# feiyeha/EGM-Unet

Measured on AMD Instinct MI355X. Metric: train images/sec at 3x512x512 bs=8/GPU, higher is better.
Workload: dtype bf16; 1 GPU; EGM-UNet GRFBUNet(3,2,base_c=32) fwd+5-term-loss+bwd+SGD, 8x3x512x512 per GPU (BASELINE.json configs[1]); global_batch=8, parallelism=dp1, launch=hipGraph replay, world_size=1

## Files before the change

### egm_unet_amd/csrc/conv3x3_wreg.hip

```cpp
#include "common.h"
#include "group.h"
#include "bn_elem.h"
#include <stdlib.h>

typedef __attribute__((ext_vector_type(8))) __bf16 bf16x8_t;
typedef __attribute__((ext_vector_type(16))) float f32x16_t;
typedef __attribute__((ext_vector_type(2))) float f32x2_t;
typedef __attribute__((ext_vector_type(2))) __bf16 bf16x2_t;

__device__ uint4 egm_dump_wreg[64];
__device__ uint4 egm_zero_page_wreg[4];

namespace {

constexpr int TW = 32, PW = TW + 2, R = 2, TROWS = 16, PH = TROWS + 2, NBUF = 3;
constexpr int PSLOTS = PH * PW * 4;
constexpr int NPI = (PSLOTS + 63) / 64;
constexpr int KT = (NPI + 7) / 8;
constexpr int STAGE = KT * 8 * 1024;
constexpr int OROW = 64 + 16;
constexpr int SMEM = NBUF * STAGE + 8 * R * 32 * OROW;
static_assert(SMEM <= 160 * 1024, "LDS budget");
static_assert(KT <= 6, "DMA slots of a stage");

struct WregParams {
    const bf16_t* x; const bf16_t* w; const float* bias; bf16_t* y; float* stats;
    int ldx, ldy, N, H, W, Cin, Cout, bias_n;
    int tiles_y, tiles_x, npt, G;
};

__device__ __forceinline__ uint32_t pack2(float lo, float hi) {
    f32x2_t v; v.x = lo; v.y = hi;
    const bf16x2_t b = __builtin_convertvector(v, bf16x2_t);
    return *reinterpret_cast<const uint32_t*>(&b);
}
__device__ __forceinline__ void glds16(const void* gsrc, unsigned lds_byte_addr) {
    unsigned keep;
    asm volatile("s_mov_b32 %0, m0\n\ts_mov_b32 m0, %2\n\ts_nop 0\n\tglobal_load_lds_dwordx4 %1, off\n\ts_mov_b32 m0, %0"
                 : "=&s"(keep) : "v"(gsrc), "s"(lds_byte_addr));
}

template <int CH>
__global__ __launch_bounds__(512, 2) void conv3x3_wreg_kernel(WregParams p) {
    constexpr int ACT = EGM_ACT_NONE;
#include "conv3x3_wreg_body.h"
}
template <int CH, int ACT>
__global__ __launch_bounds__(512, 2) void conv3x3_wreg_act_kernel(WregParams p) {
#include "conv3x3_wreg_body.h"
}

template <int CH, int ACT = EGM_ACT_NONE>
int launch_wreg(const WregParams& p, hipStream_t st) {
    constexpr auto kern = [] { if constexpr (ACT == EGM_ACT_NONE) return &conv3x3_wreg_kernel<CH>; else return &conv3x3_wreg_act_kernel<CH, ACT>; }();
    static bool attr_done = false;
    if (!attr_done) {
        hipError_t e = hipFuncSetAttribute(reinterpret_cast<const void*>(kern), hipFuncAttributeMaxDynamicSharedMemorySize, 160 * 1024);
        if (e != hipSuccess) EGM_FAIL(EGM_ERR_LAUNCH, "conv3x3_wreg: hipFuncSetAttribute: %s", hipGetErrorString(e));
        attr_done = true;
    }
    hipLaunchKernelGGL(kern, dim3(p.G), dim3(512), SMEM, st, p);
    EGM_CHECK_LAUNCH("conv3x3_wreg");
    return EGM_OK;
}
}

int egm_conv_tile_mode(int mode);

int egm_conv_wreg_plan(int dtype, int N, int H, int W, int Cin, int Cout, int KH, int KW, int dil, int* G_out) {
    if (dtype != EGM_BF16 || KH != 3 || KW != 3 || dil != 1 || Cout != 32 || Cin != 32) return 0;
    if (egm_group_recording()) return 0;
    if (!(egm_conv_tile_mode(-1) & 4)) return 0;
    const long long npt = (long long)N * egm_cdiv(H, TROWS) * egm_cdiv(W, TW);
    if (npt < 512) return 0;
    *G_out = 256;
    return 1;
}
const char* egm_conv_wreg_name(int Cin) { (void)Cin; return "conv3x3_wreg_kernel<1>"; }

int egm_conv_wreg_launch(const void* x, int ldx, const void* wf, const float* bias, int bias_n, void* y, int ldy, float* stats, int N, int H,
                         int W, int Cin, int Cout, int G, egm_stream_t s, int act) {
    WregParams p;
    p.x = (const bf16_t*)x; p.w = (const bf16_t*)wf; p.bias = bias; p.y = (bf16_t*)y; p.stats = stats;
    p.ldx = ldx; p.ldy = ldy; p.N = N; p.H = H; p.W = W; p.Cin = Cin; p.Cout = Cout; p.bias_n = bias ? bias_n : 0;
    p.tiles_y = egm_cdiv(H, TROWS); p.tiles_x = egm_cdiv(W, TW); p.npt = N * p.tiles_y * p.tiles_x; p.G = G;
    EGM_REQUIRE((long long)(PH + 1) * W * ldx < (1LL << 31), "conv3x3_wreg: halo window offsets exceed 32 bits");
    switch (act) {
        case EGM_ACT_RELU: return launch_wreg<1, EGM_ACT_RELU>(p, (hipStream_t)s);
        case EGM_ACT_SIGMOID: return launch_wreg<1, EGM_ACT_SIGMOID>(p, (hipStream_t)s);
        case EGM_ACT_SILU: return launch_wreg<1, EGM_ACT_SILU>(p, (hipStream_t)s);
        default: return launch_wreg<1>(p, (hipStream_t)s);
    }
}
```

### egm_unet_amd/csrc/conv_igemm.hip

```cpp
#include "common.h"
#include "group.h"
#include "bn_elem.h"
#include <string.h>
#include <stdio.h>

typedef __attribute__((ext_vector_type(8))) __bf16 bf16x8_t;
typedef __attribute__((ext_vector_type(16))) float f32x16_t;
typedef __attribute__((ext_vector_type(2))) unsigned short u16x2_t;

int egm_conv_direct_plan(int dtype, int N, int H, int W, int Cin, int Cout, int KH, int KW, int dil, int* NT_out, int* nct_out, int* G_out,
                         size_t* smem_out);
int egm_conv_direct_launch(const void* x, int ldx, const void* wf, const float* bias, int bias_n, void* y, int ldy,
                           float* stats, int N, int H, int W, int Cin, int Cout, int KH, int KW, int dil, int NT, int nct, int G, size_t smem,
                           egm_stream_t s, int act = EGM_ACT_NONE);

int egm_conv_tile_plan(int dtype, int N, int H, int W, int Cin, int Cout, int KH, int KW, int dil, int* cfg_out, int* nct_out, int* G_out);
const char* egm_conv_tile_name(int cfg);
int egm_conv_wreg_plan(int dtype, int N, int H, int W, int Cin, int Cout, int KH, int KW, int dil, int* G_out);
const char* egm_conv_wreg_name(int Cin);
int egm_conv_wreg_launch(const void* x, int ldx, const void* wf, const float* bias, int bias_n, void* y, int ldy, float* stats, int N, int H,
                         int W, int Cin, int Cout, int G, egm_stream_t s, int act = EGM_ACT_NONE);
int egm_conv_tile_launch(const void* x, int ldx, const void* wf, const float* bias, int bias_n, void* y, int ldy, float* stats, int N, int H,
                         int W, int Cin, int Cout, int cfg, int nct, int G, egm_stream_t s, void* y2 = nullptr, int ldy2 = 0, int csplit = 0,
                         int act = EGM_ACT_NONE);
int egm_conv_c7_plan(int dtype, int N, int H, int W, int Cin, int Cout, int KH, int KW, int dil);
int egm_conv_c7_launch(const void* x, int ldx, const void* wf, const float* bias, int bias_n, void* y, int ldy, int N, int H, int W,
                       egm_stream_t s, int act = EGM_ACT_NONE);
int egm_conv_c16d_plan(int dtype, int N, int H, int W, int Cin, int Cout, int KH, int KW, int dil);
int egm_conv_c16d_launch(const void* x, int ldx, const void* wf, const float* bias, int bias_n, void* y, int ldy, float* stats, int N, int H,
                         int W, int dil, egm_stream_t s, int act = EGM_ACT_NONE);

namespace {

constexpr int TH = 8, TW = 32, KC = 32;

template <typename T> struct Mma;
template <> struct Mma<bf16_t> {
    static constexpr int kStep = 16;
    static constexpr int kPixStride = KC * 2 + 16;
    using Frag = bf16x8_t;
    static __device__ __forceinline__ Frag load(const unsigned char* row, int ks, int h) {
        return *reinterpret_cast<const Frag*>(row + ks * 32 + h * 16);
    }
    static __device__ __forceinline__ f32x16_t mma(Frag a, Frag b, f32x16_t c) {
        return __builtin_amdgcn_mfma_f32_32x32x16_bf16(a, b, c, 0, 0, 0);
    }
    static __device__ __forceinline__ void stage16(unsigned char* dst, const bf16_t* src, bool ok) {
        uint4 v = make_uint4(0, 0, 0, 0);
        if (ok) v = *reinterpret_cast<const uint4*>(src);
        *reinterpret_cast<uint4*>(dst) = v;
    }
    static __device__ __forceinline__ void stage_val(unsigned char* dst, uint4 v) { *reinterpret_cast<uint4*>(dst) = v; }
};
template <> struct Mma<float> {
// ... 559 lines not shown
    c.R = 2;
    if (c.pipe && KH == 3 && dil == 1 && Cout <= 32) {
        const long long npt4 = (long long)N * egm_cdiv(H, 16) * egm_cdiv(W, TW);
        if (npt4 >= 256) c.R = 4;
    }
    static const int r1_on = getenv("EGM_PIPE_R1") ? atoi(getenv("EGM_PIPE_R1")) : 1;
    if (r1_on && c.pipe && KH == 3 && dil == 1 && c.R == 2 && Cout > 32 && Cin >= 128) {
        const long long wgs2 = (long long)N * egm_cdiv(H, 8) * egm_cdiv(W, TW) * egm_cdiv(Cout, 32);
        if (wgs2 <= 256) c.R = 1;
    }
    c.tiles_y = egm_cdiv(H, 4 * c.R); c.tiles_x = egm_cdiv(W, TW); c.npt = N * c.tiles_y * c.tiles_x;
    c.NT = (c.R == 4) ? (Cout <= 32 ? 1 : 2) : (c.R == 1 ? 1 : conv_nt(c.npt, Cout));
    c.nct = egm_cdiv(Cout, 32 * c.NT);
    if (!c.pipe) { c.G = c.npt; return c; }
    if (c.R == 4) {
        const int per_cu = (c.NT == 2) ? 1 : 2;
        int g = (256 * per_cu / c.nct) / 8 * 8;
        if (g < 8) g = 8;
        if (g > c.npt) g = c.npt;
        c.G = g;
    } else {
        c.G = pipe_groups(c.npt, c.nct);
    }
    return c;
}
}

extern "C" int egm_conv_kernel_name(int dtype, int N, int H, int W, int Cin, int Cout, int KH, int KW, int dil, char* buf, int buflen) {
    if (KH == 1 && KW == 1) dil = 1;
    const ConvPlan c = conv_plan(dtype, N, H, W, Cin, Cout, KH, KW, dil);
    char tmp[96];
    if (c.c16d) snprintf(tmp, sizeof(tmp), "conv3x3d_c16_kernel");
    else if (c.c7) snprintf(tmp, sizeof(tmp), "conv7x7_c16_kernel");
    else if (c.wreg) snprintf(tmp, sizeof(tmp), "%s", egm_conv_wreg_name(Cin));
    else if (c.tile) snprintf(tmp, sizeof(tmp), "%s", egm_conv_tile_name(c.tile_cfg));
    else if (c.direct) snprintf(tmp, sizeof(tmp), "conv_direct_kernel<%d, %s>", c.NT, KH == 1 ? "true" : "false");
    else if (c.pipe) snprintf(tmp, sizeof(tmp), "conv_igemm_pipe_kernel<%d, %d, %d, %d>", c.NT, (KH == 3 && dil == 1) ? 3 : 1,
                              (KH == 3 && dil == 1) ? 3 : (KH == 7 ? 7 : 1), c.R);
    else snprintf(tmp, sizeof(tmp), "conv_igemm_kernel<%s, %d>", dtype == EGM_BF16 ? "bf16_t" : "float", c.NT);
    const int n = (int)strlen(tmp);
    if (buf != nullptr && buflen > 0) { strncpy(buf, tmp, (size_t)buflen - 1); buf[buflen - 1] = 0; }
    return n;
}
extern "C" int egm_conv_stats_tiles(int dtype, int N, int H, int W, int Cin, int Cout, int KH, int KW, int dil) {
    return conv_plan(dtype, N, H, W, Cin, Cout, KH, KW, dil).G;
}

extern "C" int egm_conv_pack(int dtype, const void* w, void* wf, void* wd, int Cout, int Cin, int KH, int KW, int groups,
                             egm_stream_t s) {
    EGM_REQUIRE(w != nullptr && (wf != nullptr || wd != nullptr), "conv_pack: null pointer");
    EGM_REQUIRE(Cout > 0 && Cin > 0 && groups > 0 && Cout % groups == 0 && Cin % groups == 0, "conv_pack: bad channels/groups");
    EGM_REQUIRE(KH > 0 && KW > 0 && (KH & 1) && (KW & 1), "conv_pack: kernel must be odd");
    const int CoutP = (Cout + 7) / 8 * 8, CinP = (Cin + 7) / 8 * 8;
    const long long total = (long long)KH * KW * CoutP * CinP;
    const int grid = (int)((total + 255) / 256 > 4096 ? 4096 : (total + 255) / 256);
    EGM_DISPATCH_DTYPE(dtype, hipLaunchKernelGGL((conv_pack_kernel<T>), dim3(grid), dim3(256), 0, (hipStream_t)s,
                                                 (const float*)w, (T*)wf, (T*)wd, Cout, Cin, CoutP, CinP, KH, KW, groups));
    EGM_CHECK_LAUNCH("conv_pack");
    return EGM_OK;
}

extern "C" int egm_conv_pack_chunk(void) { return kPackChunk; }
extern "C" int egm_conv_pack_multi(int dtype, const void* table_dev, int n, long long total_chunks, egm_stream_t s) {
    EGM_REQUIRE(table_dev && n > 0 && total_chunks > 0 && total_chunks < (1LL << 30), "conv_pack_multi: bad args");
    EGM_DISPATCH_DTYPE(dtype, hipLaunchKernelGGL((conv_pack_multi_kernel<T>), dim3((unsigned)total_chunks), dim3(256), 0, (hipStream_t)s,
                                                 (const PackEntry*)table_dev, n));
    EGM_CHECK_LAUNCH("conv_pack_multi");
    return EGM_OK;
}

extern "C" int egm_conv_split_ok(int dtype, int N, int H, int W, int Cin, int Cout, int KH, int KW, int dil, int csplit) {
    if (csplit <= 0 || csplit >= Cout || csplit % 8 || N <= 0 || H <= 0 || W <= 0 || Cin <= 0 || Cin % 8 || Cout % 8) return 0;
    const ConvPlan c = conv_plan(dtype, N, H, W, Cin, Cout, KH, KW, dil);
    return (!c.c7 && !c.wreg && c.tile) ? 1 : 0;
}
extern "C" int egm_conv_fwd_split(int dtype, const void* x, int ldx, const void* wf, void* y, int ldy, void* y2, int ldy2, int csplit, int N,
                                  int H, int W, int Cin, int Cout, int KH, int KW, int dil, egm_stream_t s) {
    EGM_REQUIRE(x && wf && y && y2 && egm_aligned16(x) && egm_aligned16(wf) && egm_aligned16(y) && egm_aligned16(y2), "conv_fwd_split: bad pointers");
    EGM_REQUIRE(egm_conv_split_ok(dtype, N, H, W, Cin, Cout, KH, KW, dil, csplit), "conv_fwd_split: shape not supported (egm_conv_split_ok)");
    EGM_REQUIRE(ldx >= Cin && ldx % 8 == 0 && ldy >= csplit && ldy % 8 == 0 && ldy2 >= Cout - csplit && ldy2 % 8 == 0, "conv_fwd_split: bad ld");
    const ConvPlan c = conv_plan(dtype, N, H, W, Cin, Cout, KH, KW, dil);
    return egm_conv_tile_launch(x, ldx, wf, nullptr, 0, y, ldy, nullptr, N, H, W, Cin, Cout, c.tile_cfg, c.nct, c.G, s, y2, ldy2, csplit);
}

static int conv_fwd_impl(int dtype, const void* x, int ldx, const void* wf, const void* bias, int bias_n, void* y, int ldy, float* stats,
                         int N, int H, int W, int Cin, int Cout, int KH, int KW, int dil, int act, egm_stream_t s) {
    EGM_REQUIRE(x && wf && y, "conv_fwd: null pointer");
    EGM_REQUIRE(!bias || (bias_n > 0 && bias_n <= Cout), "conv_fwd: bad bias_n %d", bias_n);
    EGM_REQUIRE(N > 0 && H > 0 && W > 0, "conv_fwd: bad shape N=%d H=%d W=%d", N, H, W);
    EGM_REQUIRE(Cin > 0 && Cout > 0 && Cin % 8 == 0 && Cout % 8 == 0, "conv_fwd: Cin=%d/Cout=%d must be multiples of 8", Cin, Cout);
    EGM_REQUIRE(ldx >= Cin && ldy >= Cout && ldx % 8 == 0 && ldy % 8 == 0, "conv_fwd: bad ld (ldx=%d ldy=%d)", ldx, ldy);
    EGM_REQUIRE((KH & 1) && (KW & 1) && KH <= 7 && KW <= 7 && dil >= 1, "conv_fwd: unsupported kernel %dx%d dil %d", KH, KW, dil);
    EGM_REQUIRE(egm_aligned16(x) && egm_aligned16(wf) && egm_aligned16(y), "conv_fwd: pointers must be 16-byte aligned");
    EGM_REQUIRE((long long)N * H * W * (long long)(ldx > ldy ? ldx : ldy) < (1LL << 40), "conv_fwd: tensor too large");
    if (KH == 1 && KW == 1) dil = 1;

    ConvParams p;
    p.x = x; p.w = wf; p.bias = (const float*)bias; p.y = y; p.stats = stats;
    p.ldx = ldx; p.ldy = ldy; p.N = N; p.H = H; p.W = W; p.Cin = Cin; p.Cout = Cout; p.KH = KH; p.KW = KW; p.dil = dil; p.bias_n = bias ? bias_n : 0;
    p.wl = egm_w_layout(dtype, KH, KW, Cin, Cout);
    const ConvPlan c = conv_plan(dtype, N, H, W, Cin, Cout, KH, KW, dil);
    if (c.c16d) return egm_conv_c16d_launch(x, ldx, wf, (const float*)bias, bias_n, y, ldy, stats, N, H, W, dil, s, act);
    if (c.c7 && stats == nullptr) return egm_conv_c7_launch(x, ldx, wf, (const float*)bias, bias_n, y, ldy, N, H, W, s, act);
    if (c.wreg) return egm_conv_wreg_launch(x, ldx, wf, (const float*)bias, bias_n, y, ldy, stats, N, H, W, Cin, Cout, c.G, s, act);
    if (c.tile)
        return egm_conv_tile_launch(x, ldx, wf, (const float*)bias, bias_n, y, ldy, stats, N, H, W, Cin, Cout, c.tile_cfg, c.nct, c.G, s,
                                    nullptr, 0, 0, act);
    if (c.direct)
        return egm_conv_direct_launch(x, ldx, wf, (const float*)bias, bias_n, y, ldy, stats, N, H, W, Cin, Cout, KH, KW, dil, c.NT,
                                      c.nct, c.G, c.smem, s, act);
    p.tiles_y = c.tiles_y; p.tiles_x = c.tiles_x; p.npt = c.npt; p.nct = c.nct;
    const int NT = c.NT;
    if (c.pipe) {
        hipStream_t st = (hipStream_t)s;
// ... 37 lines not shown
```

### include/egm_hip.h

```cpp
#ifndef EGM_HIP_H
#define EGM_HIP_H

#ifdef __cplusplus
extern "C" {
#endif

typedef void* egm_stream_t;

enum egm_status { EGM_OK = 0, EGM_ERR_ARG = -1, EGM_ERR_LAUNCH = -2, EGM_ERR_UNSUPPORTED = -3 };
enum egm_dtype { EGM_F32 = 0, EGM_BF16 = 1 };
enum egm_act { EGM_ACT_NONE = 0, EGM_ACT_RELU = 1, EGM_ACT_SIGMOID = 2, EGM_ACT_SILU = 3  };

int egm_version(void);
const char* egm_last_error(void);
int egm_device_ok(void);

int egm_nchw_to_nhwc(int dtype, const void* src_f32, void* dst, int ld, int N, int C, int H, int W, egm_stream_t s);
int egm_nhwc_to_nchw(int dtype, const void* src, int ld, void* dst_f32, int N, int C, int H, int W, egm_stream_t s);

int egm_conv_pack(int dtype, const void* w_oihw_f32, void* wf, void* wd, int Cout, int Cin, int KH, int KW, int groups,
                  egm_stream_t s);
int egm_conv_pack_chunk(void);
int egm_conv_pack_multi(int dtype, const void* table_dev, int n, long long total_chunks, egm_stream_t s);
int egm_group_begin(void);
int egm_group_end(egm_stream_t s);
int egm_group_abort(void);
int egm_conv_tile_mode(int mode);
int egm_conv_tile_debug(int dbg);
int egm_conv_c7_mode(int mode);
int egm_conv_split_ok(int dtype, int N, int H, int W, int Cin, int Cout, int KH, int KW, int dil, int csplit);
int egm_conv_fwd_split(int dtype, const void* x, int ldx, const void* wf, void* y, int ldy, void* y2, int ldy2, int csplit, int N,
                       int H, int W, int Cin, int Cout, int KH, int KW, int dil, egm_stream_t s);
int egm_conv_kernel_name(int dtype, int N, int H, int W, int Cin, int Cout, int KH, int KW, int dil, char* buf, int buflen);
int egm_conv_fwd(int dtype, const void* x, int ldx, const void* wf, const void* bias_f32, int bias_n, void* y, int ldy,
                 float* stats, int N, int H, int W, int Cin, int Cout, int KH, int KW, int dil, egm_stream_t s);
int egm_conv_stats_tiles(int dtype, int N, int H, int W, int Cin, int Cout, int KH, int KW, int dil);
int egm_conv_fwd_act(int dtype, const void* x, int ldx, const void* wf, const void* bias_f32, int bias_n, void* y, int ldy, int N, int H,
                     int W, int Cin, int Cout, int KH, int KW, int dil, int act, egm_stream_t s);
int egm_conv_fold_chunk(void);
int egm_conv_fold_pack_multi(int dtype, const void* table_dev, int n, long long total_chunks, egm_stream_t s);
int egm_argmax_u8(const float* logits, const unsigned char* lut, unsigned char* out, int N, int C, int H, int W, egm_stream_t s);
long long egm_conv_wgrad_workspace(int N, int H, int W, int Cin, int Cout, int KH, int KW);
int egm_conv_wgrad(int dtype, const void* x, int ldx, const void* dy, int lddy, float* dw_oihw_f32, void* workspace,
                   int N, int H, int W, int Cin, int Cout, int CinR, int CoutR, int KH, int KW, int dil, int groups,
                   int accumulate, egm_stream_t s);
int egm_conv_wgrad_kernel_name(int dtype, int N, int H, int W, int Cin, int Cout, int KH, int KW, int dil, char* buf, int buflen);
#define EGM_WGRAD_MULTI_MAX 4
typedef struct egm_conv_wgrad_desc {
    const void* x; const void* dy; void* slabs;
    int ldx, lddy, N, H, W, Cin, Cout, Cin_real, Cout_real, KH, KW, dil, groups, pad_;
} egm_conv_wgrad_desc;
int egm_conv_wgrad_multi(int dtype, const egm_conv_wgrad_desc* descs, int n, egm_stream_t stream);
int egm_conv_wgrad_slabs(int dtype, int N, int H, int W, int Cin, int Cout, int KH, int KW, int dil);
int egm_wgrad_reduce(const float* slabs, float* dw_oihw_f32, int nslab, int taps, int CoutP, int CinP, int CoutR, int CinR, int groups,
                     int accumulate, egm_stream_t s);
int egm_wgrad_reduce_chunk(void);
int egm_wgrad_reduce_multi(const void* table_dev, int n, long long total_chunks, egm_stream_t s);
int egm_dwconv3_fwd(int dtype, const void* x, int ldx, const float* w, const float* b, const float* scale, void* y, int ldy,
                    int N, int H, int W, int C, egm_stream_t s);
long long egm_dwconv3_bwd_workspace(int N, int H, int W, int C);
// ... 392 lines not shown
```

Baseline: 683.7 images/s.

## Extend register-resident-weight 3x3 conv kernel to 32→64 and 64→32 channel shapes

Adds two new variants of the register-resident-weight 3x3 conv kernel. One handles Cout=64 and supports a split output; the other handles Cin=64 with 8-channel-group swizzled LDS staging. Both use an 8-row tile geometry shared through a new constexpr header. The planner now routes these shapes to the wreg path by default, with an env knob to disable it, instead of the generic tile kernels. The aim is to cut global traffic and launch overhead on the wide UNet convs, at the cost of LDS pressure and more complex DMA slot mapping that could be wrong at the edges.

After: 685.1 images/s, median of 6. Within noise of the previous version (+0.2%).

```diff
diff --git a/egm_unet_amd/csrc/conv3x3_wreg.hip b/egm_unet_amd/csrc/conv3x3_wreg.hip
--- a/egm_unet_amd/csrc/conv3x3_wreg.hip
+++ b/egm_unet_amd/csrc/conv3x3_wreg.hip
@@ -1,10 +1,12 @@
 #include "common.h"
 #include "group.h"
 #include "bn_elem.h"
+#include "conv3x3_wreg_geom.h"
 #include <stdlib.h>
 
 typedef __attribute__((ext_vector_type(8))) __bf16 bf16x8_t;
 typedef __attribute__((ext_vector_type(16))) float f32x16_t;
+typedef __attribute__((ext_vector_type(4))) float f32x4_t;
 typedef __attribute__((ext_vector_type(2))) float f32x2_t;
 typedef __attribute__((ext_vector_type(2))) __bf16 bf16x2_t;
 
@@ -50,6 +52,69 @@
 #include "conv3x3_wreg_body.h"
 }
 
+constexpr int SMEM_CO64 = NBUF * WregGeomCo64::STAGE + 8 * WregGeomCo64::R * 32 * OROW;
+static_assert(SMEM_CO64 <= 160 * 1024, "LDS budget");
+static_assert(WregGeomCo64::KT <= 6, "DMA slots of a stage");
+
+struct WregCo64Params {
+    const bf16_t* x; const bf16_t* w; const float* bias; bf16_t* y; bf16_t* y2; float* stats;
+    int ldx, ldy, ldy2, csplit, N, H, W, Cin, Cout, bias_n;
+    int tiles_y, tiles_x, npt, G;
+};
+
+template <int CH>
+__global__ __launch_bounds__(512, 2) void conv3x3_wreg_co64_kernel(WregCo64Params p) {
+    constexpr int ACT = EGM_ACT_NONE;
+#include "conv3x3_wreg_co64_body.h"
+}
+template <int CH, int ACT>
+__global__ __launch_bounds__(512, 2) void conv3x3_wreg_co64_act_kernel(WregCo64Params p) {
+#include "conv3x3_wreg_co64_body.h"
+}
+
+template <int ACT = EGM_ACT_NONE>
+int launch_wreg_co64(const WregCo64Params& p, hipStream_t st) {
+    constexpr auto kern = [] { if constexpr (ACT == EGM_ACT_NONE) return &conv3x3_wreg_co64_kernel<1>; else return &conv3x3_wreg_co64_act_kernel<1, ACT>; }();
+    static bool attr_done = false;
+    if (!attr_done) {
+        hipError_t e = hipFuncSetAttribute(reinterpret_cast<const void*>(kern), hipFuncAttributeMaxDynamicSharedMemorySize, 160 * 1024);
+        if (e != hipSuccess) EGM_FAIL(EGM_ERR_LAUNCH, "conv3x3_wreg_co64: hipFuncSetAttribute: %s", hipGetErrorString(e));
+        attr_done = true;
+    }
+    hipLaunchKernelGGL(kern, dim3(p.G), dim3(512), SMEM_CO64, st, p);
+    EGM_CHECK_LAUNCH("conv3x3_wreg_co64");
+    return EGM_OK;
+}
+
+constexpr int OROW_CI64 = 32 + 16;
+constexpr int SMEM_CI64 = NBUF * WregGeomCi64::STAGE + 1024 + 8 * WregGeomCi64::R * 32 * OROW_CI64;
+static_assert(SMEM_CI64 <= 160 * 1024, "LDS budget");
+static_assert(WregGeomCi64::KT <= 6, "DMA slots of a stage");
+
+template <int CH>
+__global__ __launch_bounds__(512, 2) void conv3x3_wreg_ci64_kernel(WregParams p) {
+    constexpr int ACT = EGM_ACT_NONE;
+#include "conv3x3_wreg_ci64_body.h"
+}
+template <int CH, int ACT>
+__global__ __launch_bounds__(512, 2) void conv3x3_wreg_ci64_act_kernel(WregParams p) {
+#include "conv3x3_wreg_ci64_body.h"
+}
+
+template <int ACT = EGM_ACT_NONE>
+int launch_wreg_ci64(const WregParams& p, hipStream_t st) {
+    constexpr auto kern = [] { if constexpr (ACT == EGM_ACT_NONE) return &conv3x3_wreg_ci64_kernel<2>; else return &conv3x3_wreg_ci64_act_kernel<2, ACT>; }();
+    static bool attr_done = false;
+    if (!attr_done) {
+        hipError_t e = hipFuncSetAttribute(reinterpret_cast<const void*>(kern), hipFuncAttributeMaxDynamicSharedMemorySize, 160 * 1024);
+        if (e != hipSuccess) EGM_FAIL(EGM_ERR_LAUNCH, "conv3x3_wreg_ci64: hipFuncSetAttribute: %s", hipGetErrorString(e));
+        attr_done = true;
+    }
+    hipLaunchKernelGGL(kern, dim3(p.G), dim3(512), SMEM_CI64, st, p);
+    EGM_CHECK_LAUNCH("conv3x3_wreg_ci64");
+    return EGM_OK;
+}
+
 template <int CH, int ACT = EGM_ACT_NONE>
 int launch_wreg(const WregParams& p, hipStream_t st) {
     constexpr auto kern = [] { if constexpr (ACT == EGM_ACT_NONE) return &conv3x3_wreg_kernel<CH>; else return &conv3x3_wreg_act_kernel<CH, ACT>; }();
@@ -67,22 +132,70 @@
 
 int egm_conv_tile_mode(int mode);
 
+static int g_wreg_wide = -1;
+extern "C" int egm_conv_wreg_wide(int on) {
+    if (g_wreg_wide < 0) {
+        const int v = getenv("EGM_WREG_WIDE") ? atoi(getenv("EGM_WREG_WIDE")) : 1;
+        g_wreg_wide = v < 0 ? 0 : v > 2 ? 2 : v;
+    }
+    const int old = g_wreg_wide;
+    if (on >= 0) g_wreg_wide = on > 2 ? 2 : on;
+    return old;
+}
+
 int egm_conv_wreg_plan(int dtype, int N, int H, int W, int Cin, int Cout, int KH, int KW, int dil, int* G_out) {
-    if (dtype != EGM_BF16 || KH != 3 || KW != 3 || dil != 1 || Cout != 32 || Cin != 32) return 0;
+    if (dtype != EGM_BF16 || KH != 3 || KW != 3 || dil != 1) return 0;
+    const bool wide = Cin != Cout;
+    if (!((Cin == 32 && Cout == 32) || (Cin == 32 && Cout == 64) || (Cin == 64 && Cout == 32))) return 0;
+    if (wide && !egm_conv_wreg_wide(-1)) return 0;
     if (egm_group_recording()) return 0;
     if (!(egm_conv_tile_mode(-1) & 4)) return 0;
-    const long long npt = (long long)N * egm_cdiv(H, TROWS) * egm_cdiv(W, TW);
+    const int trows = wide ? WregGeomCo64::TROWS : TROWS;
+    static_assert(WregGeomCo64::TROWS == WregGeomCi64::TROWS, "one tile height for both wide forms");
+    const long long npt = (long long)N * egm_cdiv(H, trows) * egm_cdiv(W, TW);
     if (npt < 512) return 0;
-    *G_out = 256;
+    if (Cin == 64 && npt < 4096 && egm_conv_wreg_wide(-1) < 2) return 0;
+    *G_out = Cin == 64 ? 512 : 256;
     return 1;
 }
-const char* egm_conv_wreg_name(int Cin) { (void)Cin; return "conv3x3_wreg_kernel<1>"; }
+const char* egm_conv_wreg_name(int Cin, int Cout) {
+    return Cout == 64 ? "conv3x3_wreg_co64_kernel<1>" : Cin == 64 ? "conv3x3_wreg_ci64_kernel<2>" : "conv3x3_wreg_kernel<1>";
+}
 
 int egm_conv_wreg_launch(const void* x, int ldx, const void* wf, const float* bias, int bias_n, void* y, int ldy, float* stats, int N, int H,
-                         int W, int Cin, int Cout, int G, egm_stream_t s, int act) {
+                         int W, int Cin, int Cout, int G, egm_stream_t s, int act, void* y2, int ldy2, int csplit) {
+    if (Cout == 64) {
+        typedef WregGeomCo64 Gm;
+        WregCo64Params p;
+        p.x = (const bf16_t*)x; p.w = (const bf16_t*)wf; p.bias = bias; p.y = (bf16_t*)y; p.stats = stats;
+        p.y2 = (bf16_t*)y2; p.ldy2 = ldy2; p.csplit = y2 ? csplit : Cout;
+        p.ldx = ldx; p.ldy = ldy; p.N = N; p.H = H; p.W = W; p.Cin = Cin; p.Cout = Cout; p.bias_n = bias ? bias_n : 0;
+        p.tiles_y = egm_cdiv(H, Gm::TROWS); p.tiles_x = egm_cdiv(W, Gm::TW); p.npt = N * p.tiles_y * p.tiles_x; p.G = G;
+        EGM_REQUIRE(p.csplit > 0 && p.csplit <= Cout && p.csplit % 8 == 0, "conv3x3_wreg_co64: bad channel split %d", p.csplit);
+        EGM_REQUIRE((long long)(Gm::PH + 1) * W * ldx < (1LL << 31), "conv3x3_wreg_co64: halo window offsets exceed 32 bits");
+        switch (act) {
+            case EGM_ACT_RELU: return launch_wreg_co64<EGM_ACT_RELU>(p, (hipStream_t)s);
+            case EGM_ACT_SIGMOID: return launch_wreg_co64<EGM_ACT_SIGMOID>(p, (hipStream_t)s);
+            case EGM_ACT_SILU: return launch_wreg_co64<EGM_ACT_SILU>(p, (hipStream_t)s);
+            default: return launch_wreg_co64<>(p, (hipStream_t)s);
+        }
+    }
+    EGM_REQUIRE(y2 == nullptr, "conv3x3_wreg: no split output for this shape");
     WregParams p;
     p.x = (const bf16_t*)x; p.w = (const bf16_t*)wf; p.bias = bias; p.y = (bf16_t*)y; p.stats = stats;
     p.ldx = ldx; p.ldy = ldy; p.N = N; p.H = H; p.W = W; p.Cin = Cin; p.Cout = Cout; p.bias_n = bias ? bias_n : 0;
+    if (Cin == 64) {
+        typedef WregGeomCi64 Gm;
+        p.tiles_y = egm_cdiv(H, Gm::TROWS); p.tiles_x = egm_cdiv(W, Gm::TW); p.npt = N * p.tiles_y * p.tiles_x;
+        p.G = G / 2;
+        EGM_REQUIRE((long long)(Gm::PH + 1) * W * ldx < (1LL << 31), "conv3x3_wreg_ci64: halo window offsets exceed 32 bits");
+        switch (act) {
+            case EGM_ACT_RELU: return launch_wreg_ci64<EGM_ACT_RELU>(p, (hipStream_t)s);
+            case EGM_ACT_SIGMOID: return launch_wreg_ci64<EGM_ACT_SIGMOID>(p, (hipStream_t)s);
+            case EGM_ACT_SILU: return launch_wreg_ci64<EGM_ACT_SILU>(p, (hipStream_t)s);
+            default: return launch_wreg_ci64<>(p, (hipStream_t)s);
+        }
+    }
     p.tiles_y = egm_cdiv(H, TROWS); p.tiles_x = egm_cdiv(W, TW); p.npt = N * p.tiles_y * p.tiles_x; p.G = G;
     EGM_REQUIRE((long long)(PH + 1) * W * ldx < (1LL << 31), "conv3x3_wreg: halo window offsets exceed 32 bits");
     switch (act) {
@@ -92,3 +205,22 @@
         default: return launch_wreg<1>(p, (hipStream_t)s);
     }
 }
+
+#define EGM_GEOM_FORM(form, expr, bad) ((form) == 0 ? [&] { typedef WregGeomCo64 Gm; return expr; }() : (form) == 1 ? [&] { typedef WregGeomCi64 Gm; return expr; }() : (bad))
+extern "C" int egm_conv_wreg_geom(int form, int* out) {
+    if (form < 0 || form > 1 || out == nullptr) return -1;
+    const int v[8] = {EGM_GEOM_FORM(form, Gm::TROWS + 0, 0), EGM_GEOM_FORM(form, Gm::PH + 0, 0), EGM_GEOM_FORM(form, Gm::PW + 0, 0), EGM_GEOM_FORM(form, Gm::NPI + 0, 0),
+                      EGM_GEOM_FORM(form, Gm::KT + 0, 0), EGM_GEOM_FORM(form, Gm::STAGE + 0, 0), EGM_GEOM_FORM(form, Gm::R + 0, 0), EGM_GEOM_FORM(form, Gm::CG + 0, 0)};
+    for (int i = 0; i < 8; ++i) out[i] = v[i];
+    return 0;
+}
+extern "C" int egm_conv_wreg_dma_slot(int form, int wv, int k, int lane, int* prow, int* col, int* group) {
+    if (form < 0 || form > 1 || wv < 0 || wv >= 8 || k < 0 || k >= EGM_GEOM_FORM(form, Gm::KT + 0, 0) || lane < 0 || lane >= 64) return -1;
+    const bool ok = EGM_GEOM_FORM(form, Gm::dma_valid(wv, k, lane), false);
+    *prow = ok ? EGM_GEOM_FORM(form, Gm::dma_prow(wv, k, lane), -1) : -1;
+    *col = ok ? EGM_GEOM_FORM(form, Gm::dma_col(wv, k, lane), -1) : -1;
+    *group = ok ? EGM_GEOM_FORM(form, Gm::dma_group(wv, k, lane), -1) : -1;
+    return EGM_GEOM_FORM(form, Gm::dma_slot(wv, k, lane), -1);
+}
+extern "C" int egm_conv_wreg_slot(int form, int prow, int col, int group) { return EGM_GEOM_FORM(form, Gm::slot(prow, col, group), -1); }
+extern "C" int egm_conv_wreg_read_slot(int form, int prow, int lane, int s, int ks, int pb) { return EGM_GEOM_FORM(form, Gm::read_slot(prow, lane, s, ks, pb), -1); }
diff --git a/egm_unet_amd/csrc/conv3x3_wreg_ci64_body.h b/egm_unet_amd/csrc/conv3x3_wreg_ci64_body.h
--- /dev/null
+++ b/egm_unet_amd/csrc/conv3x3_wreg_ci64_body.h
@@ -0,0 +1,206 @@
+    static_assert(CH == 2, "one 64-channel stage per tile");
+    typedef WregGeomCi64 Gm;
+    constexpr int PW = Gm::PW, R = Gm::R, TROWS = Gm::TROWS, KT = Gm::KT, STAGE = Gm::STAGE, TW = Gm::TW, NPI = Gm::NPI;
+    constexpr int OROW = OROW_CI64;
+    extern __shared__ __attribute__((aligned(16))) unsigned char smem[];
+    typedef __attribute__((address_space(3))) unsigned char* lds_p;
+    const int grp = blockIdx.x;
+    if (grp >= p.G) return;
+    const int tid = threadIdx.x, lane = tid & 63, r15 = lane & 15, q4 = lane >> 4;
+    const int wv = __builtin_amdgcn_readfirstlane(tid >> 6);
+    const int wr4 = wv & 3, cobase = (wv >> 2) * 16;
+    const int tpi = p.tiles_y * p.tiles_x;
+    const unsigned smem_lds = (unsigned)(unsigned long long)(lds_p)smem;
+    const void* const zp = reinterpret_cast<const void*>(egm_zero_page_wreg);
+    const bool late = wv >= 4;
+
+    int rel[KT];
+#pragma unroll
+    for (int k = 0; k < KT; ++k)
+        rel[k] = Gm::dma_valid(wv, k, lane) ? (Gm::dma_prow(wv, k, lane) * p.W + Gm::dma_col(wv, k, lane)) * p.ldx + Gm::dma_group(wv, k, lane) * 8 : -1;
+    struct Tile { int pt, n, ty, tx; };
+    const int d_n = p.G / tpi, d_rem = p.G - d_n * tpi, d_y = d_rem / p.tiles_x, d_x = d_rem - d_y * p.tiles_x;
+    auto first_tile = [&](Tile& t) {
+        t.pt = grp; t.n = grp / tpi; const int trem = grp - t.n * tpi;
+        t.ty = trem / p.tiles_x; t.tx = trem - t.ty * p.tiles_x;
+    };
+    auto next_tile = [&](Tile& t) {
+        t.pt += p.G;
+        t.tx += d_x; if (t.tx >= p.tiles_x) { t.tx -= p.tiles_x; t.ty += 1; }
+        t.ty += d_y; if (t.ty >= p.tiles_y) { t.ty -= p.tiles_y; t.n += 1; }
+        t.n += d_n;
+    };
+    struct Src { const bf16_t* xb; int oy0, ox0; unsigned lds; bool interior; };
+    auto make_src = [&](const Tile& t, int bufi) {
+        Src q;
+        q.oy0 = t.ty * TROWS; q.ox0 = t.tx * TW;
+        q.xb = p.x + ((long long)(t.n * p.H + q.oy0 - 1) * p.W + (q.ox0 - 1)) * p.ldx;
+        q.interior = q.oy0 >= 1 && q.oy0 + TROWS + 1 <= p.H && q.ox0 >= 1 && q.ox0 + TW + 1 <= p.W;
+        q.lds = smem_lds + bufi * STAGE + wv * 1024;
+        return q;
+    };
+    auto dma = [&](const Src& q, int k) __attribute__((always_inline)) {
+        bool ok = rel[k] >= 0;
+        if (!q.interior) {
+            const int prow = Gm::dma_prow(wv, k, lane), col = Gm::dma_col(wv, k, lane);
+            ok = ok && (unsigned)(q.oy0 - 1 + prow) < (unsigned)p.H && (unsigned)(q.ox0 - 1 + col) < (unsigned)p.W;
+        }
+        const void* src = ok ? reinterpret_cast<const void*>(q.xb + rel[k]) : zp;
+        glds16(src, wv + 8 * k < NPI ? q.lds + k * 8192 : smem_lds + NBUF * STAGE);
+    };
+
+    const int ntl = (p.npt - grp + p.G - 1) / p.G;
+    Tile it; first_tile(it);
+#pragma unroll
+    for (int i = 0; i < NBUF - 1; ++i) {
+        if (i < ntl) {
+            const Src q = make_src(it, i);
+#pragma unroll
+            for (int k = 0; k < KT; ++k) dma(q, k);
+            next_tile(it);
+        }
+    }
+
+    bf16x8_t wr[9][2];
+#pragma unroll
+    for (int tap = 0; tap < 9; ++tap)
+#pragma unroll
+        for (int ks = 0; ks < 2; ++ks)
+            wr[tap][ks] = *reinterpret_cast<const bf16x8_t*>(p.w + ((long long)(tap * 4 + 2 * ks + (q4 >> 1)) * p.Cout + cobase + r15) * 16 + (q4 & 1) * 8);
+    int pb[3][2];
+#pragma unroll
+    for (int s = 0; s < 3; ++s)
+#pragma unroll
+        for (int ks = 0; ks < 2; ++ks) pb[s][ks] = Gm::read_slot(R * wr4, lane, s, ks, 0) * 16;
+    static_assert(Gm::read_slot(3, 37, 2, 1, 1) == Gm::read_slot(3, 37, 2, 1, 0) + 16 * Gm::CG, "pixel block offset");
+
+    float ssum[8], ssq[8];
+    zero8(ssum); zero8(ssq);
+    unsigned char* ot = smem + NBUF * STAGE + 1024 + wv * (R * 32 * OROW);
+    unsigned char* dump = reinterpret_cast<unsigned char*>(egm_dump_wreg) + lane * 16;
+    f32x4_t acc[R][2];
+
+    auto compute = [&](int bufi, bool with_dma, const Src& q) __attribute__((always_inline)) {
+        const unsigned char* sb = smem + bufi * STAGE;
+#pragma unroll
+        for (int ks = 0; ks < 2; ++ks)
+#pragma unroll
+            for (int s = 0; s < 3; ++s) {
+#pragma unroll
+                for (int b2 = 0; b2 < 2; ++b2) {
+                    bf16x8_t fb[R + 2];
+#pragma unroll
+                    for (int rho = 0; rho < R + 2; ++rho)
+                        fb[rho] = *reinterpret_cast<const bf16x8_t*>(sb + pb[s][ks] + b2 * (16 * Gm::CG * 16) + rho * (PW * Gm::CG * 16));
+#pragma unroll
+                    for (int rho = 0; rho < R + 2; ++rho) {
+#pragma unroll
+                        for (int m = 0; m < R; ++m) {
+                            const int r = rho - m;
+                            if (r >= 0 && r < 3) acc[m][b2] = __builtin_amdgcn_mfma_f32_16x16x32_bf16(wr[r * 3 + s][ks], fb[rho], acc[m][b2], 0, 0, 0);
+                        }
+                    }
+                }
+                const int gi = ks * 3 + s;
+                if (gi < KT) {
+                    if (with_dma) dma(q, gi);
+                }
+            }
+    };
+    auto park = [&]() __attribute__((always_inline)) {
+#pragma unroll
+        for (int m = 0; m < R; ++m)
+#pragma unroll
+            for (int b2 = 0; b2 < 2; ++b2) {
+                if (p.bias != nullptr) {
+#pragma unroll
+                    for (int j = 0; j < 4; ++j) {
+                        const int co = cobase + q4 * 4 + j;
+                        acc[m][b2][j] += co < p.bias_n ? p.bias[co] : 0.f;
+                    }
+                }
+                if constexpr (ACT != EGM_ACT_NONE) {
+#pragma unroll
+                    for (int j = 0; j < 4; ++j) acc[m][b2][j] = conv_epi_act<ACT, true>(acc[m][b2][j]);
+                }
+                uint2 v;
+                v.x = pack2(acc[m][b2][0], acc[m][b2][1]);
+                v.y = pack2(acc[m][b2][2], acc[m][b2][3]);
+                *reinterpret_cast<uint2*>(ot + (m * 32 + b2 * 16 + r15) * OROW + q4 * 8) = v;
+            }
+    };
+    const int cv = lane & 1, pl = lane >> 1;
+    auto store_tile = [&](const Tile& t) __attribute__((always_inline)) {
+        const int oy0 = t.ty * TROWS, ox0 = t.tx * TW;
+        uint4 raw[R];
+#pragma unroll
+        for (int m = 0; m < R; ++m) raw[m] = *reinterpret_cast<const uint4*>(ot + (m * 32 + pl) * OROW + cv * 16);
+#pragma unroll
+        for (int m = 0; m < R; ++m) {
+            const int oy = oy0 + R * wr4 + m;
+            bf16_t* yrow = p.y + ((long long)(t.n * p.H + oy) * p.W + ox0) * p.ldy + cobase + cv * 8;
+            const bool ok = oy < p.H && ox0 + pl < p.W;
+            uint4 rw = raw[m];
+            if (!ok) rw = make_uint4(0, 0, 0, 0);
+            unsigned char* dst = ok ? reinterpret_cast<unsigned char*>(yrow + (long long)pl * p.ldy) : dump;
+            egm_store16_conv(dst, rw);
+            float v[8];
+            v[0] = __uint_as_float(rw.x << 16); v[1] = __uint_as_float(rw.x & 0xffff0000u);
+            v[2] = __uint_as_float(rw.y << 16); v[3] = __uint_as_float(rw.y & 0xffff0000u);
+            v[4] = __uint_as_float(rw.z << 16); v[5] = __uint_as_float(rw.z & 0xffff0000u);
+            v[6] = __uint_as_float(rw.w << 16); v[7] = __uint_as_float(rw.w & 0xffff0000u);
+#pragma unroll
+            for (int j = 0; j < 8; ++j) { ssum[j] += v[j]; ssq[j] = fmaf(v[j], v[j], ssq[j]); }
+        }
+    };
+
+    if (ntl > 1) asm volatile("s_waitcnt vmcnt(%0)" :: "n"(KT) : "memory");
+    else asm volatile("s_waitcnt vmcnt(0)" ::: "memory");
+    __builtin_amdgcn_s_barrier();
+    int bc = 0, bi = NBUF - 1;
+    Tile cu; first_tile(cu);
+    Tile prev = cu;
+    for (int t = 0; t < ntl; ++t) {
+        const bool more = t + NBUF - 1 < ntl;
+        const Src q = make_src(it, bi);
+        if (more) next_tile(it);
+        if (t > 0 && !late) store_tile(prev);
+#pragma unroll
+        for (int m = 0; m < R; ++m)
+#pragma unroll
+            for (int b2 = 0; b2 < 2; ++b2)
+#pragma unroll
+                for (int i = 0; i < 4; ++i) acc[m][b2][i] = 0.f;
+        compute(bc, more, q);
+        if (t > 0 && late) store_tile(prev);
+        park();
+        if (!more) asm volatile("s_waitcnt vmcnt(0)" ::: "memory");
+        else if (late && t > 0) asm volatile("s_waitcnt vmcnt(%0)" :: "n"(KT + R) : "memory");
+        else asm volatile("s_waitcnt vmcnt(%0)" :: "n"(KT) : "memory");
+        __builtin_amdgcn_s_barrier();
+        prev = cu; next_tile(cu);
+        bc = (bc + 1 == NBUF) ? 0 : bc + 1;
+        bi = (bi + 1 == NBUF) ? 0 : bi + 1;
+    }
+    store_tile(prev);
+
+    if (p.stats != nullptr) {
+#pragma unroll
+        for (int j = 0; j < 8; ++j)
+            for (int o = 2; o < 64; o <<= 1) { ssum[j] += __shfl_xor(ssum[j], o, 64); ssq[j] += __shfl_xor(ssq[j], o, 64); }
+        float* red = reinterpret_cast<float*>(smem);
+        if (lane < 2) {
+#pragma unroll
+            for (int j = 0; j < 8; ++j) { red[(wv * 2 + 0) * 16 + lane * 8 + j] = ssum[j]; red[(wv * 2 + 1) * 16 + lane * 8 + j] = ssq[j]; }
+        }
+        __syncthreads();
+        if (tid < 128) {
+            const int row = tid >> 6, which = (tid >> 5) & 1, c = tid & 31, g4 = (c >> 4) * 4, j = c & 15;
+            float v = 0.f;
+            if ((c >> 4) == row) {
+#pragma unroll
+                for (int w4 = 0; w4 < 4; ++w4) v += red[((g4 + w4) * 2 + which) * 16 + j];
+            }
+            p.stats[(((long long)grp * 2 + row) * 2 + which) * p.Cout + c] = v;
+        }
+    }
diff --git a/egm_unet_amd/csrc/conv3x3_wreg_co64_body.h b/egm_unet_amd/csrc/conv3x3_wreg_co64_body.h
--- /dev/null
+++ b/egm_unet_amd/csrc/conv3x3_wreg_co64_body.h
@@ -0,0 +1,205 @@
+    static_assert(CH == 1, "one 32-channel stage per tile");
+    typedef WregGeomCo64 Gm;
+    constexpr int PW = Gm::PW, R = Gm::R, TROWS = Gm::TROWS, KT = Gm::KT, STAGE = Gm::STAGE, TW = Gm::TW;
+    extern __shared__ __attribute__((aligned(16))) unsigned char smem[];
+    typedef __attribute__((address_space(3))) unsigned char* lds_p;
+    const int grp = blockIdx.x;
+    if (grp >= p.G) return;
+    const int tid = threadIdx.x, lane = tid & 63, r31 = lane & 31, h = lane >> 5;
+    const int wv = __builtin_amdgcn_readfirstlane(tid >> 6);
+    const int wr4 = wv & 3, cobase = (wv >> 2) * 32;
+    const int tpi = p.tiles_y * p.tiles_x;
+    const unsigned smem_lds = (unsigned)(unsigned long long)(lds_p)smem;
+    const void* const zp = reinterpret_cast<const void*>(egm_zero_page_wreg);
+    const bool late = wv >= 4;
+
+    int rel[KT];
+#pragma unroll
+    for (int k = 0; k < KT; ++k)
+        rel[k] = Gm::dma_valid(wv, k, lane) ? (Gm::dma_prow(wv, k, lane) * p.W + Gm::dma_col(wv, k, lane)) * p.ldx + Gm::dma_group(wv, k, lane) * 8 : -1;
+    struct Tile { int pt, n, ty, tx; };
+    const int d_n = p.G / tpi, d_rem = p.G - d_n * tpi, d_y = d_rem / p.tiles_x, d_x = d_rem - d_y * p.tiles_x;
+    auto first_tile = [&](Tile& t) {
+        t.pt = grp; t.n = grp / tpi; const int trem = grp - t.n * tpi;
+        t.ty = trem / p.tiles_x; t.tx = trem - t.ty * p.tiles_x;
+    };
+    auto next_tile = [&](Tile& t) {
+        t.pt += p.G;
+        t.tx += d_x; if (t.tx >= p.tiles_x) { t.tx -= p.tiles_x; t.ty += 1; }
+        t.ty += d_y; if (t.ty >= p.tiles_y) { t.ty -= p.tiles_y; t.n += 1; }
+        t.n += d_n;
+    };
+    struct Src { const bf16_t* xb; int oy0, ox0; unsigned lds; bool interior; };
+    auto make_src = [&](const Tile& t, int bufi) {
+        Src q;
+        q.oy0 = t.ty * TROWS; q.ox0 = t.tx * TW;
+        q.xb = p.x + ((long long)(t.n * p.H + q.oy0 - 1) * p.W + (q.ox0 - 1)) * p.ldx;
+        q.interior = q.oy0 >= 1 && q.oy0 + TROWS + 1 <= p.H && q.ox0 >= 1 && q.ox0 + TW + 1 <= p.W;
+        q.lds = smem_lds + bufi * STAGE + wv * 1024;
+        return q;
+    };
+    auto dma = [&](const Src& q, int k) __attribute__((always_inline)) {
+        bool ok = rel[k] >= 0;
+        if (!q.interior) {
+            const int prow = Gm::dma_prow(wv, k, lane), col = Gm::dma_col(wv, k, lane);
+            ok = ok && (unsigned)(q.oy0 - 1 + prow) < (unsigned)p.H && (unsigned)(q.ox0 - 1 + col) < (unsigned)p.W;
+        }
+        const void* src = ok ? reinterpret_cast<const void*>(q.xb + rel[k]) : zp;
+        glds16(src, q.lds + k * 8192);
+    };
+
+    const int ntl = (p.npt - grp + p.G - 1) / p.G;
+    Tile it; first_tile(it);
+#pragma unroll
+    for (int i = 0; i < NBUF - 1; ++i) {
+        if (i < ntl) {
+            const Src q = make_src(it, i);
+#pragma unroll
+            for (int k = 0; k < KT; ++k) dma(q, k);
+            next_tile(it);
+        }
+    }
+
+    bf16x8_t wr[9][2];
+#pragma unroll
+    for (int tap = 0; tap < 9; ++tap)
+#pragma unroll
+        for (int ks = 0; ks < 2; ++ks)
+            wr[tap][ks] = *reinterpret_cast<const bf16x8_t*>(p.w + ((long long)(tap * 2 + ks) * p.Cout + cobase + r31) * 16 + h * 8);
+    int pb[3][2];
+#pragma unroll
+    for (int s = 0; s < 3; ++s)
+#pragma unroll
+        for (int ks = 0; ks < 2; ++ks) pb[s][ks] = Gm::read_slot(R * wr4, lane, s, ks, 0) * 16;
+
+    float ssum[8], ssq[8];
+    zero8(ssum); zero8(ssq);
+    unsigned char* ot = smem + NBUF * STAGE + wv * (R * 32 * OROW);
+    unsigned char* dump = reinterpret_cast<unsigned char*>(egm_dump_wreg) + lane * 16;
+    f32x16_t acc[R];
+
+    auto compute = [&](int bufi, bool with_dma, const Src& q) __attribute__((always_inline)) {
+        const unsigned char* sb = smem + bufi * STAGE;
+#pragma unroll
+        for (int ks = 0; ks < 2; ++ks)
+#pragma unroll
+            for (int s = 0; s < 3; ++s) {
+                bf16x8_t fb[R + 2];
+#pragma unroll
+                for (int rho = 0; rho < R + 2; ++rho) fb[rho] = *reinterpret_cast<const bf16x8_t*>(sb + pb[s][ks] + rho * (PW * 64));
+#pragma unroll
+                for (int rho = 0; rho < R + 2; ++rho) {
+#pragma unroll
+                    for (int m = 0; m < R; ++m) {
+                        const int r = rho - m;
+                        if (r >= 0 && r < 3) acc[m] = __builtin_amdgcn_mfma_f32_32x32x16_bf16(wr[r * 3 + s][ks], fb[rho], acc[m], 0, 0, 0);
+                    }
+                }
+                const int gi = ks * 3 + s;
+                if (gi < KT) {
+                    if (with_dma) dma(q, gi);
+                }
+            }
+    };
+    auto park = [&]() __attribute__((always_inline)) {
+#pragma unroll
+        for (int m = 0; m < R; ++m)
+#pragma unroll
+            for (int gq = 0; gq < 4; ++gq) {
+                if (p.bias != nullptr) {
+#pragma unroll
+                    for (int j = 0; j < 4; ++j) {
+                        const int co = cobase + gq * 8 + h * 4 + j;
+                        acc[m][gq * 4 + j] += co < p.bias_n ? p.bias[co] : 0.f;
+                    }
+                }
+                if constexpr (ACT != EGM_ACT_NONE) {
+#pragma unroll
+                    for (int j = 0; j < 4; ++j) acc[m][gq * 4 + j] = conv_epi_act<ACT, true>(acc[m][gq * 4 + j]);
+                }
+                uint2 v;
+                v.x = pack2(acc[m][gq * 4 + 0], acc[m][gq * 4 + 1]);
+                v.y = pack2(acc[m][gq * 4 + 2], acc[m][gq * 4 + 3]);
+                *reinterpret_cast<uint2*>(ot + (m * 32 + r31) * OROW + (gq * 8 + h * 4) * 2) = v;
+            }
+    };
+    const int cv = lane & 3, slot = lane >> 2;
+    const int c0 = cobase + cv * 8;
+    bf16_t* const ych = c0 < p.csplit ? p.y + c0 : p.y2 + (c0 - p.csplit);
+    const int ldo = c0 < p.csplit ? p.ldy : p.ldy2;
+    auto store_tile = [&](const Tile& t) __attribute__((always_inline)) {
+        const int oy0 = t.ty * TROWS, ox0 = t.tx * TW;
+        uint4 raw[R][2];
+#pragma unroll
+        for (int m = 0; m < R; ++m)
+#pragma unroll
+            for (int i2 = 0; i2 < 2; ++i2) raw[m][i2] = *reinterpret_cast<const uint4*>(ot + (m * 32 + i2 * 16 + slot) * OROW + cv * 16);
+#pragma unroll
+        for (int m = 0; m < R; ++m) {
+            const int oy = oy0 + R * wr4 + m;
+            bf16_t* yrow = ych + ((long long)(t.n * p.H + oy) * p.W + ox0) * ldo;
+#pragma unroll
+            for (int i2 = 0; i2 < 2; ++i2) {
+                const int pl = i2 * 16 + slot;
+                const bool ok = oy < p.H && ox0 + pl < p.W;
+                uint4 rw = raw[m][i2];
+                if (!ok) rw = make_uint4(0, 0, 0, 0);
+                unsigned char* dst = ok ? reinterpret_cast<unsigned char*>(yrow + (long long)pl * ldo) : dump;
+                egm_store16_conv(dst, rw);
+                float v[8];
+                v[0] = __uint_as_float(rw.x << 16); v[1] = __uint_as_float(rw.x & 0xffff0000u);
+                v[2] = __uint_as_float(rw.y << 16); v[3] = __uint_as_float(rw.y & 0xffff0000u);
+                v[4] = __uint_as_float(rw.z << 16); v[5] = __uint_as_float(rw.z & 0xffff0000u);
+                v[6] = __uint_as_float(rw.w << 16); v[7] = __uint_as_float(rw.w & 0xffff0000u);
+#pragma unroll
+                for (int j = 0; j < 8; ++j) { ssum[j] += v[j]; ssq[j] = fmaf(v[j], v[j], ssq[j]); }
+            }
+        }
+    };
+
+    if (ntl > 1) asm volatile("s_waitcnt vmcnt(%0)" :: "n"(KT) : "memory");
+    else asm volatile("s_waitcnt vmcnt(0)" ::: "memory");
+    __builtin_amdgcn_s_barrier();
+    int bc = 0, bi = NBUF - 1;
+    Tile cu; first_tile(cu);
+    Tile prev = cu;
+    for (int t = 0; t < ntl; ++t) {
+        const bool more = t + NBUF - 1 < ntl;
+        const Src q = make_src(it, bi);
+        if (more) next_tile(it);
+        if (t > 0 && !late) store_tile(prev);
+#pragma unroll
+        for (int m = 0; m < R; ++m)
+#pragma unroll
+            for (int i = 0; i < 16; ++i) acc[m][i] = 0.f;
+        compute(bc, more, q);
+        if (t > 0 && late) store_tile(prev);
+        park();
+        if (!more) asm volatile("s_waitcnt vmcnt(0)" ::: "memory");
+        else if (late && t > 0) asm volatile("s_waitcnt vmcnt(%0)" :: "n"(KT + R * 2) : "memory");
+        else asm volatile("s_waitcnt vmcnt(%0)" :: "n"(KT) : "memory");
+        __builtin_amdgcn_s_barrier();
+        prev = cu; next_tile(cu);
+        bc = (bc + 1 == NBUF) ? 0 : bc + 1;
+        bi = (bi + 1 == NBUF) ? 0 : bi + 1;
+    }
+    store_tile(prev);
+
+    if (p.stats != nullptr) {
+#pragma unroll
+        for (int j = 0; j < 8; ++j)
+            for (int o = 4; o < 64; o <<= 1) { ssum[j] += __shfl_xor(ssum[j], o, 64); ssq[j] += __shfl_xor(ssq[j], o, 64); }
+        float* red = reinterpret_cast<float*>(smem);
+        if (lane < 4) {
+#pragma unroll
+            for (int j = 0; j < 8; ++j) { red[(wv * 2 + 0) * 32 + lane * 8 + j] = ssum[j]; red[(wv * 2 + 1) * 32 + lane * 8 + j] = ssq[j]; }
+        }
+        __syncthreads();
+        if (tid < 128) {
+            const int which = tid >> 6, c = tid & 63, g4 = (c >> 5) * 4, j = c & 31;
+            float v = 0.f;
+#pragma unroll
+            for (int w4 = 0; w4 < 4; ++w4) v += red[((g4 + w4) * 2 + which) * 32 + j];
+            p.stats[((long long)grp * 2 + which) * p.Cout + c] = v;
+        }
+    }
diff --git a/egm_unet_amd/csrc/conv3x3_wreg_geom.h b/egm_unet_amd/csrc/conv3x3_wreg_geom.h
--- /dev/null
+++ b/egm_unet_amd/csrc/conv3x3_wreg_geom.h
@@ -0,0 +1,28 @@
+#pragma once
+
+#if defined(__HIPCC__) || defined(__CUDACC__)
+#define EGM_GEOM_FN __host__ __device__ constexpr
+#else
+#define EGM_GEOM_FN constexpr
+#endif
+
+template <int TROWS_, int R_, int CG_>
+struct WregGeom {
+    static constexpr int TW = 32, PW = TW + 2, TROWS = TROWS_, R = R_, PH = TROWS + 2, CG = CG_;
+    static constexpr int PSLOTS = PH * PW * CG;
+    static constexpr int NPI = (PSLOTS + 63) / 64;
+    static constexpr int KT = (NPI + 7) / 8;
+    static EGM_GEOM_FN int swz(int col) { return CG == 4 ? (col >> 2) & 3 : col & 7; }
+    static EGM_GEOM_FN int slot(int prow, int col, int g) { return (prow * PW + col) * CG + (g ^ swz(col)); }
+    static EGM_GEOM_FN int dma_slot(int wv, int k, int lane) { return (wv + 8 * k) * 64 + lane; }
+    static EGM_GEOM_FN bool dma_valid(int wv, int k, int lane) { return wv + 8 * k < NPI && dma_slot(wv, k, lane) / CG < PH * PW; }
+    static EGM_GEOM_FN int dma_prow(int wv, int k, int lane) { return (dma_slot(wv, k, lane) / CG) / PW; }
+    static EGM_GEOM_FN int dma_col(int wv, int k, int lane) { return (dma_slot(wv, k, lane) / CG) % PW; }
+    static EGM_GEOM_FN int dma_group(int wv, int k, int lane) { return (dma_slot(wv, k, lane) % CG) ^ swz(dma_col(wv, k, lane)); }
+    static EGM_GEOM_FN int read_slot(int prow, int lane, int s, int ks, int pb) {
+        return CG == 4 ? slot(prow, (lane & 31) + s, 2 * ks + (lane >> 5)) : slot(prow, (lane & 15) + s + 16 * pb, 4 * ks + (lane >> 4));
+    }
+};
+
+struct WregGeomCo64 : WregGeom<8, 2, 4> { static constexpr int STAGE = KT * 8 * 1024; };
+struct WregGeomCi64 : WregGeom<8, 2, 8> { static constexpr int STAGE = NPI * 1024; };
diff --git a/egm_unet_amd/csrc/conv_igemm.hip b/egm_unet_amd/csrc/conv_igemm.hip
--- a/egm_unet_amd/csrc/conv_igemm.hip
+++ b/egm_unet_amd/csrc/conv_igemm.hip
@@ -17,9 +17,9 @@
 int egm_conv_tile_plan(int dtype, int N, int H, int W, int Cin, int Cout, int KH, int KW, int dil, int* cfg_out, int* nct_out, int* G_out);
 const char* egm_conv_tile_name(int cfg);
 int egm_conv_wreg_plan(int dtype, int N, int H, int W, int Cin, int Cout, int KH, int KW, int dil, int* G_out);
-const char* egm_conv_wreg_name(int Cin);
+const char* egm_conv_wreg_name(int Cin, int Cout);
 int egm_conv_wreg_launch(const void* x, int ldx, const void* wf, const float* bias, int bias_n, void* y, int ldy, float* stats, int N, int H,
-                         int W, int Cin, int Cout, int G, egm_stream_t s, int act = EGM_ACT_NONE);
+                         int W, int Cin, int Cout, int G, egm_stream_t s, int act = EGM_ACT_NONE, void* y2 = nullptr, int ldy2 = 0, int csplit = 0);
 int egm_conv_tile_launch(const void* x, int ldx, const void* wf, const float* bias, int bias_n, void* y, int ldy, float* stats, int N, int H,
                          int W, int Cin, int Cout, int cfg, int nct, int G, egm_stream_t s, void* y2 = nullptr, int ldy2 = 0, int csplit = 0,
                          int act = EGM_ACT_NONE);
@@ -645,7 +645,7 @@
     char tmp[96];
     if (c.c16d) snprintf(tmp, sizeof(tmp), "conv3x3d_c16_kernel");
     else if (c.c7) snprintf(tmp, sizeof(tmp), "conv7x7_c16_kernel");
-    else if (c.wreg) snprintf(tmp, sizeof(tmp), "%s", egm_conv_wreg_name(Cin));
+    else if (c.wreg) snprintf(tmp, sizeof(tmp), "%s", egm_conv_wreg_name(Cin, Cout));
     else if (c.tile) snprintf(tmp, sizeof(tmp), "%s", egm_conv_tile_name(c.tile_cfg));
     else if (c.direct) snprintf(tmp, sizeof(tmp), "conv_direct_kernel<%d, %s>", c.NT, KH == 1 ? "true" : "false");
     else if (c.pipe) snprintf(tmp, sizeof(tmp), "conv_igemm_pipe_kernel<%d, %d, %d, %d>", c.NT, (KH == 3 && dil == 1) ? 3 : 1,
@@ -685,7 +685,8 @@
 extern "C" int egm_conv_split_ok(int dtype, int N, int H, int W, int Cin, int Cout, int KH, int KW, int dil, int csplit) {
     if (csplit <= 0 || csplit >= Cout || csplit % 8 || N <= 0 || H <= 0 || W <= 0 || Cin <= 0 || Cin % 8 || Cout % 8) return 0;
     const ConvPlan c = conv_plan(dtype, N, H, W, Cin, Cout, KH, KW, dil);
-    return (!c.c7 && !c.wreg && c.tile) ? 1 : 0;
+    if (c.wreg) return Cout == 64 ? 1 : 0;
+    return (!c.c7 && c.tile) ? 1 : 0;
 }
 extern "C" int egm_conv_fwd_split(int dtype, const void* x, int ldx, const void* wf, void* y, int ldy, void* y2, int ldy2, int csplit, int N,
                                   int H, int W, int Cin, int Cout, int KH, int KW, int dil, egm_stream_t s) {
@@ -693,6 +694,7 @@
     EGM_REQUIRE(egm_conv_split_ok(dtype, N, H, W, Cin, Cout, KH, KW, dil, csplit), "conv_fwd_split: shape not supported (egm_conv_split_ok)");
     EGM_REQUIRE(ldx >= Cin && ldx % 8 == 0 && ldy >= csplit && ldy % 8 == 0 && ldy2 >= Cout - csplit && ldy2 % 8 == 0, "conv_fwd_split: bad ld");
     const ConvPlan c = conv_plan(dtype, N, H, W, Cin, Cout, KH, KW, dil);
+    if (c.wreg) return egm_conv_wreg_launch(x, ldx, wf, nullptr, 0, y, ldy, nullptr, N, H, W, Cin, Cout, c.G, s, EGM_ACT_NONE, y2, ldy2, csplit);
     return egm_conv_tile_launch(x, ldx, wf, nullptr, 0, y, ldy, nullptr, N, H, W, Cin, Cout, c.tile_cfg, c.nct, c.G, s, y2, ldy2, csplit);
 }
 
diff --git a/include/egm_hip.h b/include/egm_hip.h
--- a/include/egm_hip.h
+++ b/include/egm_hip.h
@@ -26,6 +26,7 @@
 int egm_group_end(egm_stream_t s);
 int egm_group_abort(void);
 int egm_conv_tile_mode(int mode);
+int egm_conv_wreg_wide(int on);
 int egm_conv_tile_debug(int dbg);
 int egm_conv_c7_mode(int mode);
 int egm_conv_split_ok(int dtype, int N, int H, int W, int Cin, int Cout, int KH, int KW, int dil, int csplit);
```
